# MarSaKi/VLN-BEVBert

Measured on AMD Instinct MI355X. Metric: pretrain_samples_per_sec, higher is better.
Workload: dtype bf16+fp32-residual

## Files before the change

### vln_bevbert_amd/csrc/attn_fwd2.hip

```cpp
#include "attn_mfma_common.h"

#define FWD2_THR 5.0f

typedef const __attribute__((address_space(4))) uint64_t* bb_cu64p;

__device__ __forceinline__ float drop_select(float p, uint64_t lane_mask) {
  return __builtin_amdgcn_inverse_ballot_w64(lane_mask) ? p : 0.f;
}
__device__ __forceinline__ float max3f(float a, float b, float c) { return fmaxf(fmaxf(a, b), c); }

#define F2_LD 72
#define F2_TILE (TK * F2_LD)
__device__ __forceinline__ int f2_off(int row, int chunk) { return row * F2_LD + (chunk << 3); }
__device__ __forceinline__ bf16x8 f2_frag_rows(const bf16_raw* tile, int t, int ks, int lane) {
  return as_bf16x8(*reinterpret_cast<const uint4*>(tile + f2_off(t * 16 + (lane & 15), ks * 4 + (lane >> 4))));
}
__device__ __forceinline__ bf16x8 f2_frag_tr(const bf16_raw* img, int row_lo, int row_hi, int col0, int lane) {
  const int i = lane & 15, col = col0 + 4 * (i & 3);
  const int rl = row_lo + (i >> 2), rh = row_hi + (i >> 2);
  const uint2 lo = lds_tr16(img + f2_off(rl, col >> 3) + (col & 7));
  const uint2 hi = lds_tr16(img + f2_off(rh, col >> 3) + (col & 7));
  return as_bf16x8(make_uint4(lo.x, lo.y, hi.x, hi.y));
}

template <int NW, bool DROP>
__global__ __launch_bounds__(64 * NW, 4) void attn_fwd2_kernel(AttnArgs a) {
  constexpr int QT = 2;
  constexpr int NT = 64 * NW;
  constexpr int CPT = (512 + NT - 1) / NT;
  __shared__ __attribute__((aligned(16))) bf16_raw s_k[2][F2_TILE];
  __shared__ __attribute__((aligned(16))) bf16_raw s_v[2][F2_TILE];
  __shared__ __attribute__((aligned(16))) float s_mask[2][TK];
  const int tid = threadIdx.x, lane = tid & 63, g = lane >> 4, c = lane & 15;
  const int w = __builtin_amdgcn_readfirstlane(tid >> 6);
  int blk, h, b;
  attn_decode_block(a, blk, h, b);
  const int qbase = blk * (16 * QT * NW) + w * (16 * QT);
  const bf16_raw* qp = (const bf16_raw*)a.q + (size_t)b * a.bsq + h * ATTN_D;
  const bf16_raw* kp = (const bf16_raw*)a.k + (size_t)b * a.bsk + h * ATTN_D;
  const bf16_raw* vp = (const bf16_raw*)a.v + (size_t)b * a.bsv + h * ATTN_D;
  const float sc2 = a.scale * LOG2E;
  const float inv_scale = 1.0f / a.scale;

  bf16x8 qf[QT][2];
  int qrow[QT];
#pragma unroll
  for (int qt = 0; qt < QT; ++qt) {
    qrow[qt] = qbase + qt * 16 + c;
    const int r = qrow[qt] < a.Lq ? qrow[qt] : a.Lq - 1;
#pragma unroll
    for (int ks = 0; ks < 2; ++ks) qf[qt][ks] = as_bf16x8(ld_frag_global(qp, a.ldq, r, ks * 32 + g * 8));
  }
  bb_cu64p wq[QT];
  if (DROP) {
#pragma unroll
    for (int qt = 0; qt < QT; ++qt) {
      int q16 = (qbase >> 4) + qt;
      q16 = q16 < a.nq16 ? q16 : a.nq16 - 1;
      wq[qt] = (bb_cu64p)(uintptr_t)(a.drop_bits + ((size_t)(b * a.nh + h) * a.nq16 + q16) * a.nk64 * 16);
    }
  }
  f32x4 oacc[QT][4];
  float m_run[QT], nm[QT], l_run[QT];
#pragma unroll
  for (int qt = 0; qt < QT; ++qt) {
    m_run[qt] = -INFINITY;
    nm[qt] = 0.f;
    l_run[qt] = 0.f;
#pragma unroll
    for (int dt = 0; dt < 4; ++dt) oacc[qt][dt] = (f32x4){0.f, 0.f, 0.f, 0.f};
  }

  auto mask_of = [&](int kv0) -> float {
    const int key = kv0 + tid;
    if (tid >= TK || key >= a.Lk) return -INFINITY;
    return a.key_mask ? a.key_mask[(size_t)b * a.Lk + key] * inv_scale : 0.f;
  };
  uint4 kreg[CPT], vreg[CPT];
  float mreg;
  auto stage_load = [&](int kv0) {
#pragma unroll
    for (int i = 0; i < CPT; ++i) {
      const int ch = tid + i * NT, row = ch >> 3, d0 = (ch & 7) * 8;
      kreg[i] = vreg[i] = make_uint4(0, 0, 0, 0);
      if (ch < 512 && kv0 + row < a.Lk) {
        kreg[i] = ld_frag_global(kp, a.ldk, kv0 + row, d0);
        vreg[i] = ld_frag_global(vp, a.ldv, kv0 + row, d0);
      }
    }
    mreg = mask_of(kv0);
  };
  auto stage_store = [&](int buf) {
#pragma unroll
    for (int i = 0; i < CPT; ++i) {
      const int ch = tid + i * NT, row = ch >> 3, d0 = (ch & 7) * 8;
      if (ch < 512) {
        *reinterpret_cast<uint4*>(s_k[buf] + f2_off(row, ch & 7)) = kreg[i];
        *reinterpret_cast<uint4*>(s_v[buf] + f2_off(row, ch & 7)) = vreg[i];
      }
    }
    if (tid < TK) s_mask[buf][tid] = mreg;
  };
  stage_load(0);
  stage_store(0);
  if (TK < a.Lk) stage_load(TK);
  __syncthreads();

  uint64_t kw[8];
#pragma unroll
  for (int i = 0; i < 8; ++i) kw[i] = DROP ? wq[0][i] : 0;
  for (int kv0 = 0, cur = 0; kv0 < a.Lk; kv0 += TK, cur ^= 1) {
    const bf16_raw* ck = s_k[cur];
    const bf16_raw* cv = s_v[cur];
    const float* cmask = s_mask[cur];
#pragma unroll
    for (int hh = 0; hh < 2; ++hh) {
      f32x4 sacc[QT][2];
#pragma unroll
      for (int tt = 0; tt < 2; ++tt) {
        const int t = 2 * hh + tt;
        const float4 mk = *reinterpret_cast<const float4*>(&cmask[t * 16 + g * 4]);
#pragma unroll
        for (int qt = 0; qt < QT; ++qt) sacc[qt][tt] = (f32x4){mk.x, mk.y, mk.z, mk.w};
#pragma unroll
        for (int ks = 0; ks < 2; ++ks) {
          const bf16x8 kf = f2_frag_rows(ck, t, ks, lane);
#pragma unroll
          for (int qt = 0; qt < QT; ++qt) sacc[qt][tt] = mfma16(kf, qf[qt][ks], sacc[qt][tt]);
        }
      }
      if (hh == 0 && kv0 + TK < a.Lk) {
        stage_store(cur ^ 1);
        if (kv0 + 2 * TK < a.Lk) stage_load(kv0 + 2 * TK);
      }
      float lm[QT];
      bool grow = false;
#pragma unroll
      for (int qt = 0; qt < QT; ++qt) {
        const f32x4 s0 = sacc[qt][0], s1 = sacc[qt][1];
        lm[qt] = max3f(max3f(s0[0], s0[1], s0[2]), max3f(s0[3], s1[0], s1[1]), fmaxf(s1[2], s1[3])) * sc2;
        grow |= lm[qt] > m_run[qt] + FWD2_THR;
      }
      if (__any(grow)) {
#pragma unroll
        for (int qt = 0; qt < QT; ++qt) {
          const float m_new = fmaxf(m_run[qt], quad_max(lm[qt]));
          const float nm_new = (m_new == -INFINITY) ? 0.f : -m_new;
          const float alpha = fast_exp2(m_run[qt] + nm_new);
          m_run[qt] = m_new;
          nm[qt] = nm_new;
          l_run[qt] *= alpha;
#pragma unroll
          for (int dt = 0; dt < 4; ++dt) oacc[qt][dt] *= alpha;
        }
      }
      bf16x8 pb[QT];
#pragma unroll
      for (int qt = 0; qt < QT; ++qt) {
        uint64_t kwn[8];
        if (DROP) {
          const int kvn = (qt + 1 < QT || hh == 0) ? kv0 : (kv0 + TK < a.Lk ? kv0 + TK : kv0);
          const int hn = qt + 1 < QT ? hh : hh ^ 1, qn = qt + 1 < QT ? qt + 1 : 0;
#pragma unroll
          for (int i = 0; i < 8; ++i) kwn[i] = wq[qn][(kvn >> 6) * 16 + hn * 8 + i];
          __builtin_amdgcn_sched_barrier(0);
        }
        float psum = 0.f;
#pragma unroll
        for (int tt = 0; tt < 2; ++tt)
#pragma unroll
          for (int r = 0; r < 4; ++r) {
            float p = fast_exp2(fmaf(sacc[qt][tt][r], sc2, nm[qt]));
            psum += p;
            if (DROP) p = drop_select(p, kw[tt * 4 + r]);
            sacc[qt][tt][r] = p;
          }
        l_run[qt] += psum;
        pb[qt] = pack_pair(sacc[qt][0], sacc[qt][1]);
        if (DROP) {
#pragma unroll
          for (int i = 0; i < 8; ++i) kw[i] = kwn[i];
        }
      }
#pragma unroll
      for (int dt = 0; dt < 4; ++dt) {
        const bf16x8 vf = f2_frag_tr(cv, 32 * hh + 4 * g, 32 * hh + 16 + 4 * g, dt * 16, lane);
#pragma unroll
        for (int qt = 0; qt < QT; ++qt) oacc[qt][dt] = mfma16(vf, pb[qt], oacc[qt][dt]);
      }

    }
    __syncthreads();
  }

  const float ks = DROP ? a.keep_scale : 1.0f;
#pragma unroll
  for (int qt = 0; qt < QT; ++qt) {
    const float l = quad_sum(l_run[qt]);
    const float inv = ks / l;
    if (qrow[qt] < a.Lq) {
      bf16_raw* op = (bf16_raw*)a.o + (size_t)b * a.bso + (size_t)qrow[qt] * a.ldo + h * ATTN_D;
#pragma unroll
      for (int dt = 0; dt < 4; ++dt)
        st4<bf16_raw>(op + dt * 16 + g * 4, make_float4(oacc[qt][dt][0] * inv, oacc[qt][dt][1] * inv,
                                                         oacc[qt][dt][2] * inv, oacc[qt][dt][3] * inv));
      if (a.lse && g == 0) a.lse[((size_t)b * a.nh + h) * a.Lq + qrow[qt]] = (log2f(l) - nm[qt]) * LN2;
    }
  }
}

template <int NW, bool DROP, int ABL = 0>
__global__ __launch_bounds__(64 * NW, 4) void attn_fwd3_kernel(AttnArgs a) {
  constexpr int QT = 2;
  constexpr int NT = 64 * NW;
  constexpr int CPT = (512 + NT - 1) / NT;
  __shared__ __attribute__((aligned(16))) bf16_raw s_k[2][F2_TILE];
  __shared__ __attribute__((aligned(16))) bf16_raw s_v[2][F2_TILE];
  __shared__ __attribute__((aligned(16))) float s_mask[2][TK];
  const int tid = threadIdx.x, lane = tid & 63, g = lane >> 4, c = lane & 15;
  const int w = __builtin_amdgcn_readfirstlane(tid >> 6);
  int blk, h, b;
  attn_decode_block(a, blk, h, b);
  const int qbase = blk * (16 * QT * NW) + w * (16 * QT);
  const bf16_raw* qp = (const bf16_raw*)a.q + (size_t)b * a.bsq + h * ATTN_D;
  const bf16_raw* kp = (const bf16_raw*)a.k + (size_t)b * a.bsk + h * ATTN_D;
  const bf16_raw* vp = (const bf16_raw*)a.v + (size_t)b * a.bsv + h * ATTN_D;
  const float sc2 = a.scale * LOG2E;
  const float inv_scale = 1.0f / a.scale;

  bf16x8 qf[QT][2];
  int qrow[QT];
#pragma unroll
  for (int qt = 0; qt < QT; ++qt) {
    qrow[qt] = qbase + qt * 16 + c;
    const int r = qrow[qt] < a.Lq ? qrow[qt] : a.Lq - 1;
#pragma unroll
    for (int ks = 0; ks < 2; ++ks) qf[qt][ks] = as_bf16x8(ld_frag_global(qp, a.ldq, r, ks * 32 + g * 8));
  }
  bb_cu64p wq[QT];
  if (DROP) {
#pragma unroll
    for (int qt = 0; qt < QT; ++qt) {
      int q16 = (qbase >> 4) + qt;
      q16 = q16 < a.nq16 ? q16 : a.nq16 - 1;
      wq[qt] = (bb_cu64p)(uintptr_t)(a.drop_bits + ((size_t)(b * a.nh + h) * a.nq16 + q16) * a.nk64 * 16);
    }
  }
  f32x4 oacc[QT][4];
  float m_run[QT], nm[QT], l_run[QT];
#pragma unroll
  for (int qt = 0; qt < QT; ++qt) {
    m_run[qt] = -INFINITY;
    nm[qt] = 0.f;
    l_run[qt] = 0.f;
#pragma unroll
    for (int dt = 0; dt < 4; ++dt) oacc[qt][dt] = (f32x4){0.f, 0.f, 0.f, 0.f};
  }

  auto mask_of = [&](int kv0) -> float {
    const int key = kv0 + tid;
    if (tid >= TK || key >= a.Lk) return -INFINITY;
    return a.key_mask ? a.key_mask[(size_t)b * a.Lk + key] * inv_scale : 0.f;
  };
  uint4 kreg[CPT], vreg[CPT];
  float mreg;
  auto stage_load = [&](int kv0) {
#pragma unroll
    for (int i = 0; i < CPT; ++i) {
      const int ch = tid + i * NT, row = ch >> 3, d0 = (ch & 7) * 8;
      kreg[i] = vreg[i] = make_uint4(0, 0, 0, 0);
      if (ch < 512 && kv0 + row < a.Lk) {
        kreg[i] = ld_frag_global(kp, a.ldk, kv0 + row, d0);
        vreg[i] = ld_frag_global(vp, a.ldv, kv0 + row, d0);
      }
    }
    mreg = mask_of(kv0);
  };
  auto stage_store = [&](int buf) {
#pragma unroll
    for (int i = 0; i < CPT; ++i) {
      const int ch = tid + i * NT, row = ch >> 3, d0 = (ch & 7) * 8;
      if (ch < 512) {
        *reinterpret_cast<uint4*>(s_k[buf] + f2_off(row, ch & 7)) = kreg[i];
        *reinterpret_cast<uint4*>(s_v[buf] + f2_off(row, ch & 7)) = vreg[i];
      }
    }
    if (tid < TK) s_mask[buf][tid] = mreg;
  };
  stage_load(0);
  stage_store(0);
  if (TK < a.Lk) stage_load(TK);
  __syncthreads();

  uint64_t kw[QT][16];
#pragma unroll
  for (int qt = 0; qt < QT; ++qt)
#pragma unroll
    for (int i = 0; i < 16; ++i) kw[qt][i] = DROP ? wq[qt][i] : 0;
  const int Lk_run = (ABL & 64) ? (a.Lk < TK ? a.Lk : TK) : a.Lk;
  for (int kv0 = 0, cur = 0; kv0 < Lk_run; kv0 += TK, cur ^= 1) {
    const bf16_raw* ck = s_k[cur];
    const bf16_raw* cv = s_v[cur];
    const float* cmask = s_mask[cur];
#pragma unroll
    for (int hh = 0; hh < 2; ++hh) {
      f32x4 sacc[QT][2];
#pragma unroll
      for (int tt = 0; tt < 2; ++tt) {
        const int t = 2 * hh + tt;
        const float4 mk = *reinterpret_cast<const float4*>(&cmask[t * 16 + g * 4]);
#pragma unroll
        for (int qt = 0; qt < QT; ++qt) sacc[qt][tt] = (f32x4){mk.x, mk.y, mk.z, mk.w};
#pragma unroll
        for (int ks = 0; ks < 2; ++ks) {
          const bf16x8 kf = f2_frag_rows(ck, t, ks, lane);
#pragma unroll
          for (int qt = 0; qt < QT; ++qt) if (!(ABL & 4)) sacc[qt][tt] = mfma16(kf, qf[qt][ks], sacc[qt][tt]);
        }
      }
      if (hh == 0 && kv0 + TK < a.Lk && !((ABL & 8) && kv0 > 0)) {
        stage_store(cur ^ 1);
        if (kv0 + 2 * TK < a.Lk) stage_load(kv0 + 2 * TK);
      }
#pragma unroll
      for (int qt = 0; qt < QT; ++qt)
#pragma unroll
        for (int tt = 0; tt < 2; ++tt)
#pragma unroll
          for (int r = 0; r < 4; ++r) sacc[qt][tt][r] = fmaf(sacc[qt][tt][r], sc2, nm[qt]);
      float lm[QT];
      bool grow = false;
#pragma unroll
      for (int qt = 0; qt < QT; ++qt) {
        const f32x4 s0 = sacc[qt][0], s1 = sacc[qt][1];
        lm[qt] = max3f(max3f(s0[0], s0[1], s0[2]), max3f(s0[3], s1[0], s1[1]), fmaxf(s1[2], s1[3]));
        grow |= (lm[qt] > FWD2_THR) | ((m_run[qt] == -INFINITY) & (lm[qt] > -INFINITY));
      }
      if ((ABL & 16) ? (kv0 == 0 && hh == 0) : __any(grow)) {
#pragma unroll
        for (int qt = 0; qt < QT; ++qt) {
          const float m_new = fmaxf(m_run[qt], quad_max(lm[qt]) - nm[qt]);
          const float nm_new = (m_new == -INFINITY) ? 0.f : -m_new;
          const float alpha = fast_exp2(m_run[qt] + nm_new);
          const float shift = nm_new - nm[qt];
          m_run[qt] = m_new;
          nm[qt] = nm_new;
          l_run[qt] *= alpha;
#pragma unroll
          for (int dt = 0; dt < 4; ++dt) oacc[qt][dt] *= alpha;
#pragma unroll
          for (int tt = 0; tt < 2; ++tt)
#pragma unroll
            for (int r = 0; r < 4; ++r) sacc[qt][tt][r] += shift;
        }
      }
      bf16x8 pb[QT];
#pragma unroll
      for (int qt = 0; qt < QT; ++qt) {
        float psum = 0.f;
#pragma unroll
        for (int tt = 0; tt < 2; ++tt)
#pragma unroll
          for (int r = 0; r < 4; ++r) {
            float p = (ABL & 1) ? sacc[qt][tt][r] : fast_exp2(sacc[qt][tt][r]);
            psum += p;
            if (DROP && !(ABL & 1)) {
              p = drop_select(p, kw[qt][(2 * hh + tt) * 4 + r]);
              asm("" : "+v"(p));
            }
            sacc[qt][tt][r] = p;
          }
        l_run[qt] += psum;
        pb[qt] = pack_pair(sacc[qt][0], sacc[qt][1]);
      }
#pragma unroll
      for (int dt = 0; dt < 4; ++dt) {
        const bf16x8 vf = f2_frag_tr(cv, 32 * hh + 4 * g, 32 * hh + 16 + 4 * g, dt * 16, lane);
#pragma unroll
        for (int qt = 0; qt < QT; ++qt) if (!(ABL & 2)) oacc[qt][dt] = mfma16(vf, pb[qt], oacc[qt][dt]);
      }

    }
    __builtin_amdgcn_sched_barrier(0);
    if (DROP) {
      const int kvn = kv0 + TK < a.Lk ? kv0 + TK : kv0;
      bb_cu64p w0 = wq[0] + (kvn >> 6) * 16, w1 = wq[1] + (kvn >> 6) * 16;
      asm volatile("s_waitcnt lgkmcnt(0)" : "+s"(w0), "+s"(w1) : : "memory");
#pragma unroll
      for (int i = 0; i < 16; ++i) { kw[0][i] = w0[i]; kw[1][i] = w1[i]; }
    } else {
      asm volatile("s_waitcnt lgkmcnt(0)" : : : "memory");
    }
    __builtin_amdgcn_s_barrier();
    asm volatile("" : : : "memory");
  }

  const float ks = DROP ? a.keep_scale : 1.0f;
#pragma unroll
  for (int qt = 0; qt < QT; ++qt) {
    const float l = quad_sum(l_run[qt]);
    const float inv = ks / l;
    if (qrow[qt] < a.Lq) {
      bf16_raw* op = (bf16_raw*)a.o + (size_t)b * a.bso + (size_t)qrow[qt] * a.ldo + h * ATTN_D;
#pragma unroll
      for (int dt = 0; dt < 4; ++dt)
        st4<bf16_raw>(op + dt * 16 + g * 4, make_float4(oacc[qt][dt][0] * inv, oacc[qt][dt][1] * inv,
                                                         oacc[qt][dt][2] * inv, oacc[qt][dt][3] * inv));
      if (a.lse && g == 0) a.lse[((size_t)b * a.nh + h) * a.Lq + qrow[qt]] = (log2f(l) - nm[qt]) * LN2;
    }
  }
}

template <int LANE0> __device__ __forceinline__ void put_words4(uint32_t& lo, uint32_t& hi, uint64_t m0, uint64_t m1,
                                                              uint64_t m2, uint64_t m3) {
  asm volatile("s_nop 3\n\t"
               "v_writelane_b32 %0, %2, %10\n\tv_writelane_b32 %1, %3, %10\n\t"
               "v_writelane_b32 %0, %4, %11\n\tv_writelane_b32 %1, %5, %11\n\t"
               "v_writelane_b32 %0, %6, %12\n\tv_writelane_b32 %1, %7, %12\n\t"
               "v_writelane_b32 %0, %8, %13\n\tv_writelane_b32 %1, %9, %13"
               : "+v"(lo), "+v"(hi)
               : "s"((uint32_t)m0), "s"((uint32_t)(m0 >> 32)), "s"((uint32_t)m1), "s"((uint32_t)(m1 >> 32)),
                 "s"((uint32_t)m2), "s"((uint32_t)(m2 >> 32)), "s"((uint32_t)m3), "s"((uint32_t)(m3 >> 32)),
                 "n"(LANE0), "n"(LANE0 + 1), "n"(LANE0 + 2), "n"(LANE0 + 3));
}

template <bool WITH_B>
__global__ __launch_bounds__(256) void attn_drop_bits_kernel(AttnArgs a, uint64_t* bits_f, uint64_t* bits_b, uint32_t* bits_l) {
  constexpr int NQT = WITH_B ? 4 : 1;
  const int lane = threadIdx.x & 63, g = lane >> 4, c = lane & 15;
  const int wave = blockIdx.x * 4 + (threadIdx.x >> 6), nwaves = gridDim.x * 4;
  const uint32_t key = bb_salted(a.drop_key, a.salt);
  const uint32_t thr_hi = a.drop_thr << 16;
  const int nqg = a.nq16 / NQT, per_bh = nqg * a.nk64, total = a.B * a.nh * per_bh;
  for (int gtask = wave; gtask < total; gtask += nwaves) {
    const int bh = gtask / per_bh, rem = gtask - bh * per_bh, qg = rem / a.nk64, k64 = rem - qg * a.nk64;
    uint32_t wl0 = 0, wl1 = 0;
#pragma unroll 1
   for (int qt = 0; qt < NQT; ++qt) {
    const int q16 = qg * NQT + qt;
    const int task = (bh * a.nq16 + q16) * a.nk64 + k64;
    const int q = q16 * 16 + c;
    const uint32_t rbase = (uint32_t)(((uint32_t)bh * a.Lq + (q < a.Lq ? q : a.Lq - 1)) * (uint32_t)a.Lk2);
    uint32_t mine = 0;
    uint32_t flo = 0, fhi = 0;
#pragma unroll
    for (int t = 0; t < 4; ++t) {
      const uint32_t pr = (rbase + (uint32_t)(k64 * 64 + t * 16 + g * 4)) >> 1;
      const uint32_t b0 = bb_pair_bits(key, pr), b1 = bb_pair_bits(key, pr + 1);
      const bool k0 = (b0 << 16) >= thr_hi, k1 = b0 >= thr_hi, k2 = (b1 << 16) >= thr_hi, k3 = b1 >= thr_hi;
      const uint64_t m0 = __ballot(k0), m1 = __ballot(k1), m2 = __ballot(k2), m3 = __ballot(k3);
      if (t == 0) put_words4<0>(flo, fhi, m0, m1, m2, m3);
      if (t == 1) put_words4<4>(flo, fhi, m0, m1, m2, m3);
      if (t == 2) put_words4<8>(flo, fhi, m0, m1, m2, m3);
      if (t == 3) put_words4<12>(flo, fhi, m0, m1, m2, m3);
      if (WITH_B) {
        const uint32_t nib = (k0 ? 1u : 0u) | (k1 ? 2u : 0u) | (k2 ? 4u : 0u) | (k3 ? 8u : 0u);
        mine |= nib << (4 * t);
      }
    }
    if (lane < 16) bits_f[(size_t)task * 16 + lane] = ((uint64_t)fhi << 32) | flo;
    if (WITH_B) {
      uint32_t blo = 0, bhi = 0;
      uint32_t got[4];
#pragma unroll
      for (int rp = 0; rp < 4; ++rp)
        got[rp] = (uint32_t)__builtin_amdgcn_ds_bpermute(((c >> 2) * 16 + 4 * g + rp) << 2, (int)mine) >> (c & 3);
#define BB_B_WORDS(T) put_words4<4 * T>(blo, bhi, __ballot((got[0] >> (4 * T)) & 1u), __ballot((got[1] >> (4 * T)) & 1u), \
                                        __ballot((got[2] >> (4 * T)) & 1u), __ballot((got[3] >> (4 * T)) & 1u));
      BB_B_WORDS(0) BB_B_WORDS(1) BB_B_WORDS(2) BB_B_WORDS(3)
#undef BB_B_WORDS
      if (lane < 16) {
        const int t = lane >> 2, rp = lane & 3;
        const size_t wi = ((((size_t)bh * (a.nq16 >> 1) + (q16 >> 1)) * a.nk64 + k64) * 2 + (q16 & 1)) * 16 + t * 4 + rp;
        bits_b[wi] = ((uint64_t)bhi << 32) | blo;
      }
      uint32_t ev = mine & 0x5555u, od = (mine >> 1) & 0x5555u;
      ev = (ev | (ev >> 1)) & 0x3333u; od = (od | (od >> 1)) & 0x3333u;
      ev = (ev | (ev >> 2)) & 0x0f0fu; od = (od | (od >> 2)) & 0x0f0fu;
      ev = (ev | (ev >> 4)) & 0x00ffu; od = (od | (od >> 4)) & 0x00ffu;
      wl0 |= ((ev & 15u) | ((od & 15u) << 16)) << (4 * qt);
      wl1 |= ((ev >> 4) | ((od >> 4) << 16)) << (4 * qt);
    }
   }
    if (WITH_B) {
      uint32_t* dst = bits_l + (((size_t)bh * nqg + qg) * a.nk64 + k64) * 128 + lane;
      dst[0] = wl0;
      dst[64] = wl1;
    }
  }
}

int attn_drop_bits(const AttnArgs& a, uint64_t* bits_f, uint64_t* bits_b, uint32_t* bits_l, hipStream_t st) {
  const bool with_b = bits_b != nullptr && bits_l != nullptr && a.bias == nullptr && a.Lk > 256 && a.Lk <= 448;
  const int total = a.B * a.nh * (with_b ? a.nq16 / 4 : a.nq16) * a.nk64;
  int nb = (total + 3) / 4;
  if (nb > 8192) nb = 8192;
  if (with_b) hipLaunchKernelGGL(attn_drop_bits_kernel<true>, dim3(nb), dim3(256), 0, st, a, bits_f, bits_b, bits_l);
  else hipLaunchKernelGGL(attn_drop_bits_kernel<false>, dim3(nb), dim3(256), 0, st, a, bits_f, bits_b, bits_l);
  BB_CHECK_LAUNCH("attn_drop_bits");
  return BB_OK;
}

template <int NW>
static int launch_fwd2(const AttnArgs& a_in, hipStream_t st) {
  AttnArgs a = a_in;
  a.nblk = (a.Lq + 32 * NW - 1) / (32 * NW);
  const dim3 grid((unsigned)a.nblk * a.nh * a.B);
  static const int var = [] { const char* v = getenv("BEVBERT_FWD_VAR"); return v ? atoi(v) : 1; }();
  if (var == 0) {
    if (a.drop_p > 0.f) hipLaunchKernelGGL((attn_fwd2_kernel<NW, true>), grid, dim3(64 * NW), 0, st, a);
    else hipLaunchKernelGGL((attn_fwd2_kernel<NW, false>), grid, dim3(64 * NW), 0, st, a);
  } else {
    static const int abl = [] { const char* v = getenv("BEVBERT_FWD_ABL"); return v ? atoi(v) : 0; }();
    if (abl && a.drop_p > 0.f && NW == 4) {
      switch (abl) {
        case 1: hipLaunchKernelGGL((attn_fwd3_kernel<4, true, 1>), grid, dim3(256), 0, st, a); return BB_OK;
        case 2: hipLaunchKernelGGL((attn_fwd3_kernel<4, true, 2>), grid, dim3(256), 0, st, a); return BB_OK;
        case 4: hipLaunchKernelGGL((attn_fwd3_kernel<4, true, 4>), grid, dim3(256), 0, st, a); return BB_OK;
        case 6: hipLaunchKernelGGL((attn_fwd3_kernel<4, true, 6>), grid, dim3(256), 0, st, a); return BB_OK;
        case 7: hipLaunchKernelGGL((attn_fwd3_kernel<4, true, 7>), grid, dim3(256), 0, st, a); return BB_OK;
        case 8: hipLaunchKernelGGL((attn_fwd3_kernel<4, true, 8>), grid, dim3(256), 0, st, a); return BB_OK;
        case 16: hipLaunchKernelGGL((attn_fwd3_kernel<4, true, 16>), grid, dim3(256), 0, st, a); return BB_OK;
        case 17: hipLaunchKernelGGL((attn_fwd3_kernel<4, true, 17>), grid, dim3(256), 0, st, a); return BB_OK;
        case 31: hipLaunchKernelGGL((attn_fwd3_kernel<4, true, 31>), grid, dim3(256), 0, st, a); return BB_OK;
        case 64: hipLaunchKernelGGL((attn_fwd3_kernel<4, true, 64>), grid, dim3(256), 0, st, a); return BB_OK;
        case 95: hipLaunchKernelGGL((attn_fwd3_kernel<4, true, 95>), grid, dim3(256), 0, st, a); return BB_OK;
        default: break;
      }
    }
    if (a.drop_p > 0.f) hipLaunchKernelGGL((attn_fwd3_kernel<NW, true>), grid, dim3(64 * NW), 0, st, a);
    else hipLaunchKernelGGL((attn_fwd3_kernel<NW, false>), grid, dim3(64 * NW), 0, st, a);
  }
  BB_CHECK_LAUNCH("attn_fwd(mfma, gen 2)");
  return BB_OK;
}

bool attn_fwd2_supported(const AttnArgs& a) { return a.bias == nullptr && (a.drop_p <= 0.f || a.drop_bits != nullptr); }

int attn_fwd2(const AttnArgs& a, hipStream_t st) {
  BB_REQUIRE(attn_mfma_operands_aligned(a, false), "attention (MFMA path): " ATTN_MFMA_ALIGN_MSG);
  static const int force = [] { const char* v = getenv("BEVBERT_FWD2_NW"); return v ? atoi(v) : 0; }();
  if (force == 7) return launch_fwd2<7>(a, st);
  if (force == 8) return launch_fwd2<8>(a, st);
  return launch_fwd2<4>(a, st);
}
```

### vln_bevbert_amd/csrc/splat.hip

```cpp
#include "common.h"

#define MAX_CELLS 1024
#define MAX_POINTS 24576

struct LiftArgs {
  const float* depths;
  const float* T_c2w;
  const float* T_w2c;
  const float* S_w2c;
  const float* pix;
  const float* points;
  const uint8_t* pmask;
  int V, hw;
  float depth_scale;
  int P, dim;
  float res, half, y_clip;
  int* cell;
  int* order;
  int* cell_start;
};

__device__ __forceinline__ int cell_of(float ex, float ey, float ez, bool dropped, int dim, float res, float half,
                                       float y_clip) {
  const float fx = rintf(__fadd_rn(__fdiv_rn(ex, res), half));
  const float fz = rintf(__fadd_rn(__fdiv_rn(ez, res), half));
  const float fd = (float)dim;
  const bool outside = (fx >= fd) | (fz >= fd) | (fx < 0.f) | (fz < 0.f);
  if (dropped | outside | (ey > y_clip)) return -1;
  return dim * (int)fz + (int)fx;
}

#define LIFT_WAVES 16
#define LIFT_THREADS (LIFT_WAVES * 64)
template <int MODE>
__global__ __launch_bounds__(LIFT_THREADS) void bev_bin_sort_kernel(LiftArgs a) {
  __shared__ short s_cell[MAX_POINTS];
  __shared__ int s_cnt[MAX_CELLS + 1];
  const int b = blockIdx.x, tid = threadIdx.x;
  const int K = a.dim * a.dim;
  for (int c = tid; c <= K; c += LIFT_THREADS) s_cnt[c] = 0;
  __syncthreads();

  for (int p = tid; p < a.P; p += LIFT_THREADS) {
    int cid;
    if (MODE == 0) {
      const int hw2 = a.hw * a.hw;
      const int v = p / hw2, r = (p - v * hw2) / a.hw, u = p % a.hw;
      const float z = __fmul_rn(a.depths[(size_t)b * a.P + p], a.depth_scale);
      const float x = __fmul_rn(z, a.pix[u]);
      const float y = __fmul_rn(z, a.pix[r]);
      const float* T = a.T_c2w + ((size_t)b * a.V + v) * 16;
      float w[3];
#pragma unroll
      for (int i = 0; i < 3; ++i)
        w[i] = __fadd_rn(__fadd_rn(__fadd_rn(__fmul_rn(T[i * 4 + 0], x), __fmul_rn(T[i * 4 + 1], y)),
                                   __fmul_rn(T[i * 4 + 2], z)),
                         T[i * 4 + 3]);
      const float* S = a.S_w2c + (size_t)b * 3;
      const float p0 = __fsub_rn(w[0], S[0]), p1 = __fsub_rn(w[1], S[1]), p2 = __fsub_rn(w[2], S[2]);
      const float* R = a.T_w2c + (size_t)b * 16;
      float e[3];
#pragma unroll
      for (int i = 0; i < 3; ++i)
        e[i] = __fadd_rn(__fadd_rn(__fadd_rn(__fmul_rn(R[i * 4 + 0], p0), __fmul_rn(R[i * 4 + 1], p1)),
                                   __fmul_rn(R[i * 4 + 2], p2)),
                         R[i * 4 + 3]);
      cid = cell_of(e[0], e[1], e[2], z == 0.f, a.dim, a.res, a.half, a.y_clip);
    } else {
      const float* q = a.points + ((size_t)b * a.P + p) * 3;
      cid = cell_of(q[0], q[1], q[2], a.pmask[(size_t)b * a.P + p] != 0, a.dim, a.res, a.half, a.y_clip);
    }
    s_cell[p] = (short)cid;
    a.cell[(size_t)b * a.P + p] = cid;
    if (cid >= 0) atomicAdd(&s_cnt[cid], 1);
  }
  __syncthreads();

  if (tid < 64) {
    const int per = (K + 63) / 64;
    const int c0 = tid * per;
    int sum = 0;
    for (int i = 0; i < per; ++i)
      if (c0 + i < K) sum += s_cnt[c0 + i];
    int incl = sum;
#pragma unroll
    for (int o = 1; o < 64; o <<= 1) {
      int t = __shfl_up(incl, o, 64);
      if (tid >= o) incl += t;
    }
    int run = incl - sum;
    for (int i = 0; i < per; ++i)
      if (c0 + i < K) {
        const int n = s_cnt[c0 + i];
        s_cnt[c0 + i] = run;
        run += n;
      }
    if (tid == 63) s_cnt[K] = incl;
  }
  __syncthreads();
  for (int c = tid; c <= K; c += LIFT_THREADS) a.cell_start[(size_t)b * (K + 1) + c] = s_cnt[c];

  __shared__ int s_wbase[LIFT_WAVES][MAX_CELLS + 1];
  const int lane = tid & 63, wv = tid >> 6;
  for (int c = tid; c < LIFT_WAVES * (MAX_CELLS + 1); c += LIFT_THREADS) (&s_wbase[0][0])[c] = 0;
  __syncthreads();
  const int per_wave = ((a.P + LIFT_THREADS - 1) / LIFT_THREADS) * 64;
  const int pw0 = wv * per_wave;
  for (int p = pw0 + lane; p < pw0 + per_wave && p < a.P; p += 64) {
    const int cid = s_cell[p];
    if (cid >= 0) atomicAdd(&s_wbase[wv][cid], 1);
  }
  __syncthreads();
  for (int c = tid; c < K; c += LIFT_THREADS) {
    int base = s_cnt[c];
#pragma unroll
    for (int w = 0; w < LIFT_WAVES; ++w) {
      const int n = s_wbase[w][c];
      s_wbase[w][c] = base;
      base += n;
    }
  }
  __syncthreads();
  int* dst = a.order + (size_t)b * a.P;
  const unsigned long long lt = lane == 0 ? 0ull : (~0ull >> (64 - lane));
  for (int p0 = pw0; p0 < pw0 + per_wave && p0 < a.P; p0 += 64) {
    const int p = p0 + lane;
    const int cid = p < a.P ? (int)s_cell[p] : -1;
    unsigned long long todo = __ballot(cid >= 0);
    while (todo) {
      const int leader = __builtin_ctzll(todo);
      const int c0 = __shfl(cid, leader, 64);
      const unsigned long long same = __ballot(cid == c0);
      const int base = s_wbase[wv][c0];
      if (cid == c0) dst[base + __builtin_popcountll(same & lt)] = p;
      if (lane == leader) s_wbase[wv][c0] = base + __builtin_popcountll(same);
      todo &= ~same;
    }
  }
}

template <typename TI, typename TO>
__global__ __launch_bounds__(256) void bev_splat_mean_kernel(const TI* __restrict__ feat, const int* __restrict__ order,
                                                             const int* __restrict__ cell_start, TO* __restrict__ out,
                                                             int P, int K, int C,
                                                             const uint8_t* __restrict__ sem_ids,
                                                             const double* __restrict__ sem_dense,
                                                             int S, uint8_t* __restrict__ out_sem,
                                                             uint8_t* __restrict__ out_sem_mask,
                                                             const int* __restrict__ sample_rows,
                                                             int R) {
  const int cellg = blockIdx.x;
  const int b = cellg / K, cell = cellg - b * K;
  const int P0 = P / R;
  const int* rows = sample_rows != nullptr ? sample_rows + (size_t)b * R : nullptr;
  auto src_point = [&](int p) -> size_t {
    if (rows == nullptr) return (size_t)b * P + p;
    if (R == 1) return (size_t)rows[0] * P0 + p;
    const int r = p / P0;
    return (size_t)rows[r] * P0 + (p - r * P0);
  };
  const int s0 = cell_start[(size_t)b * (K + 1) + cell];
  const int n = cell_start[(size_t)b * (K + 1) + cell + 1] - s0;
  const int* ord = order + (size_t)b * P + s0;
  const float inv_denominator = (float)(n > 1 ? n : 1);

  for (int c4 = threadIdx.x; c4 * 4 < C; c4 += blockDim.x) {
    float4 acc = make_float4(0.f, 0.f, 0.f, 0.f);
    int i = 0;
    for (; i + 4 <= n; i += 4) {
      const int p0 = ord[i], p1 = ord[i + 1], p2 = ord[i + 2], p3 = ord[i + 3];
      const float4 v0 = ld4<TI>(feat + src_point(p0) * C + c4 * 4);
      const float4 v1 = ld4<TI>(feat + src_point(p1) * C + c4 * 4);
      const float4 v2 = ld4<TI>(feat + src_point(p2) * C + c4 * 4);
      const float4 v3 = ld4<TI>(feat + src_point(p3) * C + c4 * 4);
      acc.x = __fadd_rn(__fadd_rn(__fadd_rn(__fadd_rn(acc.x, v0.x), v1.x), v2.x), v3.x);
      acc.y = __fadd_rn(__fadd_rn(__fadd_rn(__fadd_rn(acc.y, v0.y), v1.y), v2.y), v3.y);
      acc.z = __fadd_rn(__fadd_rn(__fadd_rn(__fadd_rn(acc.z, v0.z), v1.z), v2.z), v3.z);
      acc.w = __fadd_rn(__fadd_rn(__fadd_rn(__fadd_rn(acc.w, v0.w), v1.w), v2.w), v3.w);
    }
    for (; i < n; ++i) {
      const float4 v = ld4<TI>(feat + src_point(ord[i]) * C + c4 * 4);
      acc.x = __fadd_rn(acc.x, v.x); acc.y = __fadd_rn(acc.y, v.y);
      acc.z = __fadd_rn(acc.z, v.z); acc.w = __fadd_rn(acc.w, v.w);
    }
    acc.x = __fdiv_rn(acc.x, inv_denominator); acc.y = __fdiv_rn(acc.y, inv_denominator);
    acc.z = __fdiv_rn(acc.z, inv_denominator); acc.w = __fdiv_rn(acc.w, inv_denominator);
    st4<TO>(out + (size_t)cellg * C + c4 * 4, acc);
  }

  if (out_sem != nullptr) {
    int any = 0;
    for (int c = threadIdx.x; c < S; c += blockDim.x) {
      uint8_t flag = 0;
      if (sem_ids != nullptr) {
        for (int i = 0; i < n; ++i) flag |= (uint8_t)(sem_ids[src_point(ord[i])] == (uint8_t)c);
      } else {
        const double* sb = sem_dense + (size_t)b * P * S;
        double acc = 0.0;
        for (int i = 0; i < n; ++i) acc += sb[(size_t)ord[i] * S + c];
        flag = (uint8_t)(acc / (double)(n > 1 ? n : 1) > 0.0);
      }
      out_sem[(size_t)cellg * S + c] = flag;
      any |= flag;
    }
    any = __syncthreads_or(any);
    if (threadIdx.x == 0) out_sem_mask[cellg] = (uint8_t)(any != 0);
  }
}

BEVBERT_API int bevbert_bev_lift_bin(const float* depths, const float* T_c2w, const float* T_w2c, const float* S_w2c,
                                     const float* pix_scale, int B, int V, int hw, float depth_scale, int dim,
                                     float res, float y_clip, int* cell, int* order, int* cell_start,
                                     hipStream_t stream) {
  const int P = V * hw * hw;
  BB_REQUIRE(B > 0 && P > 0 && P <= MAX_POINTS, "bev_lift_bin: P=%d out of range (max %d)", P, MAX_POINTS);
  BB_REQUIRE(dim > 0 && dim * dim <= MAX_CELLS, "bev_lift_bin: dim=%d too large", dim);
  LiftArgs a;
  memset(&a, 0, sizeof(a));
  a.depths = depths; a.T_c2w = T_c2w; a.T_w2c = T_w2c; a.S_w2c = S_w2c; a.pix = pix_scale;
  a.V = V; a.hw = hw; a.depth_scale = depth_scale; a.P = P; a.dim = dim; a.res = res;
  a.half = (float)(dim - 1) / 2.0f; a.y_clip = y_clip;
  a.cell = cell; a.order = order; a.cell_start = cell_start;
  hipLaunchKernelGGL(bev_bin_sort_kernel<0>, dim3(B), dim3(LIFT_THREADS), 0, stream, a);
  BB_CHECK_LAUNCH("bev_lift_bin");
  return BB_OK;
}

BEVBERT_API int bevbert_bev_bin_points(const float* points, const uint8_t* drop_mask, int B, int P, int dim, float res,
                                       float y_clip, int* cell, int* order, int* cell_start, hipStream_t stream) {
  BB_REQUIRE(B > 0 && P > 0 && P <= MAX_POINTS, "bev_bin_points: P=%d out of range (max %d)", P, MAX_POINTS);
  BB_REQUIRE(dim > 0 && dim * dim <= MAX_CELLS, "bev_bin_points: dim=%d too large", dim);
  LiftArgs a;
  memset(&a, 0, sizeof(a));
  a.points = points; a.pmask = drop_mask; a.P = P; a.dim = dim; a.res = res;
  a.half = (float)(dim - 1) / 2.0f; a.y_clip = y_clip;
  a.cell = cell; a.order = order; a.cell_start = cell_start;
  hipLaunchKernelGGL(bev_bin_sort_kernel<1>, dim3(B), dim3(LIFT_THREADS), 0, stream, a);
  BB_CHECK_LAUNCH("bev_bin_points");
  return BB_OK;
}

template <typename TI, typename TO>
static int launch_splat(const void* feat, const int* order, const int* cell_start, void* out, int B, int P, int K,
                        int C, const uint8_t* sem_ids, const double* sem_dense, int S, uint8_t* out_sem,
                        uint8_t* out_sem_mask, const int* sample_rows, int R, hipStream_t stream) {
  const int threads = (C / 4 >= 192) ? 192 : ((C / 4 + 63) / 64) * 64;
  hipLaunchKernelGGL((bev_splat_mean_kernel<TI, TO>), dim3(B * K), dim3(threads < 64 ? 64 : threads), 0, stream,
                     (const TI*)feat, order, cell_start, (TO*)out, P, K, C, sem_ids, sem_dense, S, out_sem,
                     out_sem_mask, sample_rows, R);
  BB_CHECK_LAUNCH("bev_splat_mean");
  return BB_OK;
}

BEVBERT_API int bevbert_bev_splat_mean(const void* feat, int feat_dtype, const int* order, const int* cell_start,
                                       void* out, int out_dtype, int B, int P, int K, int C, const uint8_t* sem_ids,
                                       const double* sem_dense, int S, uint8_t* out_sem, uint8_t* out_sem_mask,
                                       const int* sample_rows, int rows_per_sample, hipStream_t stream) {
  BB_REQUIRE(C % 4 == 0, "bev_splat_mean: C=%d must be a multiple of 4", C);
  const int R = rows_per_sample < 1 ? 1 : rows_per_sample;
  BB_REQUIRE(R == 1 || sample_rows != nullptr, "bev_splat_mean: rows_per_sample=%d needs sample_rows", R);
  BB_REQUIRE(P % R == 0, "bev_splat_mean: P=%d is not a multiple of rows_per_sample=%d", P, R);
  BB_REQUIRE(sample_rows == nullptr || sem_dense == nullptr,
             "bev_splat_mean: sample_rows indexes feat / sem_ids stores; dense semantics are per batch");
  BB_REQUIRE(out_sem == nullptr || (sem_ids != nullptr) != (sem_dense != nullptr),
             "bev_splat_mean: exactly one of sem_ids / sem_dense when semantics are requested");
#define GO(TI, TO) \
  return launch_splat<TI, TO>(feat, order, cell_start, out, B, P, K, C, sem_ids, sem_dense, S, out_sem, out_sem_mask, sample_rows, R, stream)
  if (feat_dtype == BB_F32 && out_dtype == BB_F32) GO(float, float);
  if (feat_dtype == BB_F32 && out_dtype == BB_BF16) GO(float, bf16_raw);
  if (feat_dtype == BB_BF16 && out_dtype == BB_F32) GO(bf16_raw, float);
  if (feat_dtype == BB_BF16 && out_dtype == BB_BF16) GO(bf16_raw, bf16_raw);
  if (feat_dtype == BB_F16 && out_dtype == BB_F32) GO(_Float16, float);
  if (feat_dtype == BB_F16 && out_dtype == BB_BF16) GO(_Float16, bf16_raw);
  if (feat_dtype == BB_F16 && out_dtype == BB_F16) GO(_Float16, _Float16);
#undef GO
  bb_set_error("bev_splat_mean: unsupported dtype pair (%d -> %d)", feat_dtype, out_dtype);
  return BB_EUNSUPPORTED;
}
```

Baseline: 3703.

## Parallelize BEV bin-sort across point chunks and streamline dropout-bit packing

The BEV bin-sort kernel now launches one block per (batch, point chunk) rather than one block per batch. Each block recomputes cell ids for all points to get global counts, then ranks its own points inside each wave by intersecting one ballot per cell-id bit, and scatters the order entries directly. This trades redundant per-block cell computation for much more parallelism than a single block per sample. Separately, the attention dropout-bit kernel's WITH_B path is restructured: transposed and lane-packed masks are built with carry-add lane-bit accumulation and bpermute plus bit-swizzles, replacing per-tile ballots and shift cascades.

Result: no change. 3694 (-0.3%).

```diff
diff --git a/vln_bevbert_amd/csrc/attn_fwd2.hip b/vln_bevbert_amd/csrc/attn_fwd2.hip
--- a/vln_bevbert_amd/csrc/attn_fwd2.hip
+++ b/vln_bevbert_amd/csrc/attn_fwd2.hip
@@ -424,6 +424,80 @@
                  "n"(LANE0), "n"(LANE0 + 1), "n"(LANE0 + 2), "n"(LANE0 + 3));
 }
 
+template <int LANE0> __device__ __forceinline__ void put_words4_lane_bits(uint32_t& lo, uint32_t& hi, uint32_t& ev, uint32_t& od,
+                                                                        uint64_t m0, uint64_t m1, uint64_t m2, uint64_t m3) {
+  asm volatile("s_nop 3\n\t"
+               "v_writelane_b32 %[lo], %[m0l], %[l0]\n\tv_writelane_b32 %[hi], %[m0h], %[l0]\n\t"
+               "v_writelane_b32 %[lo], %[m1l], %[l1]\n\tv_writelane_b32 %[hi], %[m1h], %[l1]\n\t"
+               "v_writelane_b32 %[lo], %[m2l], %[l2]\n\tv_writelane_b32 %[hi], %[m2h], %[l2]\n\t"
+               "v_writelane_b32 %[lo], %[m3l], %[l3]\n\tv_writelane_b32 %[hi], %[m3h], %[l3]\n\t"
+               "v_addc_co_u32_e64 %[od], vcc, %[od], %[od], %[m3]\n\t"
+               "v_addc_co_u32_e64 %[ev], vcc, %[ev], %[ev], %[m2]\n\t"
+               "v_addc_co_u32_e64 %[od], vcc, %[od], %[od], %[m1]\n\t"
+               "v_addc_co_u32_e64 %[ev], vcc, %[ev], %[ev], %[m0]"
+               : [lo] "+v"(lo), [hi] "+v"(hi), [ev] "+v"(ev), [od] "+v"(od)
+               : [m0l] "s"((uint32_t)m0), [m0h] "s"((uint32_t)(m0 >> 32)), [m1l] "s"((uint32_t)m1),
+                 [m1h] "s"((uint32_t)(m1 >> 32)), [m2l] "s"((uint32_t)m2), [m2h] "s"((uint32_t)(m2 >> 32)),
+                 [m3l] "s"((uint32_t)m3), [m3h] "s"((uint32_t)(m3 >> 32)), [m0] "s"(m0), [m1] "s"(m1), [m2] "s"(m2),
+                 [m3] "s"(m3), [l0] "n"(LANE0), [l1] "n"(LANE0 + 1), [l2] "n"(LANE0 + 2), [l3] "n"(LANE0 + 3)
+               : "vcc");
+}
+
+template <int QT, int T>
+__device__ __forceinline__ void drop_bits_step(uint32_t key, uint32_t thr_hi, uint32_t elem0, uint32_t& flo, uint32_t& fhi,
+                                               uint32_t& ev, uint32_t& od) {
+  const uint32_t pr = (elem0 + (uint32_t)(T * 16)) >> 1;
+  const uint32_t b0 = bb_pair_bits(key, pr), b1 = bb_pair_bits(key, pr + 1);
+  const bool k0 = (b0 << 16) >= thr_hi, k1 = b0 >= thr_hi, k2 = (b1 << 16) >= thr_hi, k3 = b1 >= thr_hi;
+  put_words4_lane_bits<16 * QT + 4 * T>(flo, fhi, ev, od, __ballot(k0), __ballot(k1), __ballot(k2), __ballot(k3));
+}
+
+template <int QT>
+__device__ __forceinline__ void drop_bits_tile(const AttnArgs& a, uint32_t key, uint32_t thr_hi, int bh, int q16, int k64,
+                                               int g, int c, uint32_t& flo, uint32_t& fhi, uint32_t (&acc)[2][2]) {
+  const int q = q16 * 16 + c;
+  const uint32_t rbase = (uint32_t)(((uint32_t)bh * a.Lq + (q < a.Lq ? q : a.Lq - 1)) * (uint32_t)a.Lk2);
+  const uint32_t elem0 = rbase + (uint32_t)(k64 * 64 + g * 4);
+  drop_bits_step<QT, 3>(key, thr_hi, elem0, flo, fhi, acc[1][0], acc[1][1]);
+  drop_bits_step<QT, 2>(key, thr_hi, elem0, flo, fhi, acc[1][0], acc[1][1]);
+  drop_bits_step<QT, 1>(key, thr_hi, elem0, flo, fhi, acc[0][0], acc[0][1]);
+  drop_bits_step<QT, 0>(key, thr_hi, elem0, flo, fhi, acc[0][0], acc[0][1]);
+}
+
+__device__ __forceinline__ void drop_bits_task_fbl(const AttnArgs& a, uint32_t key, uint32_t thr_hi, int bh, int qg, int k64,
+                                                   int lane, uint64_t* bits_f, uint64_t* bits_b, uint32_t* bits_l) {
+  const int g = lane >> 4, c = lane & 15;
+  uint32_t flo = 0, fhi = 0;
+  uint32_t acc[2][2] = {{0, 0}, {0, 0}};
+  drop_bits_tile<3>(a, key, thr_hi, bh, qg * 4 + 3, k64, g, c, flo, fhi, acc);
+  drop_bits_tile<2>(a, key, thr_hi, bh, qg * 4 + 2, k64, g, c, flo, fhi, acc);
+  drop_bits_tile<1>(a, key, thr_hi, bh, qg * 4 + 1, k64, g, c, flo, fhi, acc);
+  drop_bits_tile<0>(a, key, thr_hi, bh, qg * 4 + 0, k64, g, c, flo, fhi, acc);
+  const int q16 = qg * 4 + g, j = c;
+  const int task = (bh * a.nq16 + q16) * a.nk64 + k64;
+  bits_f[(size_t)task * 16 + j] = ((uint64_t)fhi << 32) | flo;
+
+  const int rp = lane & 3, quad = (lane & ~3) << 2;
+  uint32_t xlo = 0, xhi = 0;
+#pragma unroll
+  for (int i = 0; i < 4; ++i) {
+    const uint32_t slo = (uint32_t)__builtin_amdgcn_ds_bpermute(quad + 4 * i, (int)flo);
+    const uint32_t shi = (uint32_t)__builtin_amdgcn_ds_bpermute(quad + 4 * i, (int)fhi);
+    xlo |= ((slo >> rp) & 0x11111111u) << i;
+    xhi |= ((shi >> rp) & 0x11111111u) << i;
+  }
+  uint64_t x = ((uint64_t)xhi << 32) | xlo;
+  uint64_t sw = ((x >> 12) ^ x) & 0x0000F0F00000F0F0ull;
+  x ^= sw ^ (sw << 12);
+  sw = ((x >> 24) ^ x) & 0x00000000FF00FF00ull;
+  x ^= sw ^ (sw << 24);
+  const size_t wi = ((((size_t)bh * (a.nq16 >> 1) + (q16 >> 1)) * a.nk64 + k64) * 2 + (q16 & 1)) * 16 + j;
+  bits_b[wi] = x;
+  uint32_t* dst = bits_l + (((size_t)bh * (a.nq16 / 4) + qg) * a.nk64 + k64) * 128 + lane;
+  dst[0] = acc[0][0] | (acc[0][1] << 16);
+  dst[64] = acc[1][0] | (acc[1][1] << 16);
+}
+
 template <bool WITH_B>
 __global__ __launch_bounds__(256) void attn_drop_bits_kernel(AttnArgs a, uint64_t* bits_f, uint64_t* bits_b, uint32_t* bits_l) {
   constexpr int NQT = WITH_B ? 4 : 1;
@@ -434,14 +508,13 @@
   const int nqg = a.nq16 / NQT, per_bh = nqg * a.nk64, total = a.B * a.nh * per_bh;
   for (int gtask = wave; gtask < total; gtask += nwaves) {
     const int bh = gtask / per_bh, rem = gtask - bh * per_bh, qg = rem / a.nk64, k64 = rem - qg * a.nk64;
-    uint32_t wl0 = 0, wl1 = 0;
-#pragma unroll 1
-   for (int qt = 0; qt < NQT; ++qt) {
-    const int q16 = qg * NQT + qt;
-    const int task = (bh * a.nq16 + q16) * a.nk64 + k64;
-    const int q = q16 * 16 + c;
+    if (WITH_B) {
+      drop_bits_task_fbl(a, key, thr_hi, bh, qg, k64, lane, bits_f, bits_b, bits_l);
+      continue;
+    }
+    const int task = (bh * a.nq16 + qg) * a.nk64 + k64;
+    const int q = qg * 16 + c;
     const uint32_t rbase = (uint32_t)(((uint32_t)bh * a.Lq + (q < a.Lq ? q : a.Lq - 1)) * (uint32_t)a.Lk2);
-    uint32_t mine = 0;
     uint32_t flo = 0, fhi = 0;
 #pragma unroll
     for (int t = 0; t < 4; ++t) {
@@ -453,40 +526,8 @@
       if (t == 1) put_words4<4>(flo, fhi, m0, m1, m2, m3);
       if (t == 2) put_words4<8>(flo, fhi, m0, m1, m2, m3);
       if (t == 3) put_words4<12>(flo, fhi, m0, m1, m2, m3);
-      if (WITH_B) {
-        const uint32_t nib = (k0 ? 1u : 0u) | (k1 ? 2u : 0u) | (k2 ? 4u : 0u) | (k3 ? 8u : 0u);
-        mine |= nib << (4 * t);
-      }
     }
     if (lane < 16) bits_f[(size_t)task * 16 + lane] = ((uint64_t)fhi << 32) | flo;
-    if (WITH_B) {
-      uint32_t blo = 0, bhi = 0;
-      uint32_t got[4];
-#pragma unroll
-      for (int rp = 0; rp < 4; ++rp)
-        got[rp] = (uint32_t)__builtin_amdgcn_ds_bpermute(((c >> 2) * 16 + 4 * g + rp) << 2, (int)mine) >> (c & 3);
-#define BB_B_WORDS(T) put_words4<4 * T>(blo, bhi, __ballot((got[0] >> (4 * T)) & 1u), __ballot((got[1] >> (4 * T)) & 1u), \
-                                        __ballot((got[2] >> (4 * T)) & 1u), __ballot((got[3] >> (4 * T)) & 1u));
-      BB_B_WORDS(0) BB_B_WORDS(1) BB_B_WORDS(2) BB_B_WORDS(3)
-#undef BB_B_WORDS
-      if (lane < 16) {
-        const int t = lane >> 2, rp = lane & 3;
-        const size_t wi = ((((size_t)bh * (a.nq16 >> 1) + (q16 >> 1)) * a.nk64 + k64) * 2 + (q16 & 1)) * 16 + t * 4 + rp;
-        bits_b[wi] = ((uint64_t)bhi << 32) | blo;
-      }
-      uint32_t ev = mine & 0x5555u, od = (mine >> 1) & 0x5555u;
-      ev = (ev | (ev >> 1)) & 0x3333u; od = (od | (od >> 1)) & 0x3333u;
-      ev = (ev | (ev >> 2)) & 0x0f0fu; od = (od | (od >> 2)) & 0x0f0fu;
-      ev = (ev | (ev >> 4)) & 0x00ffu; od = (od | (od >> 4)) & 0x00ffu;
-      wl0 |= ((ev & 15u) | ((od & 15u) << 16)) << (4 * qt);
-      wl1 |= ((ev >> 4) | ((od >> 4) << 16)) << (4 * qt);
-    }
-   }
-    if (WITH_B) {
-      uint32_t* dst = bits_l + (((size_t)bh * nqg + qg) * a.nk64 + k64) * 128 + lane;
-      dst[0] = wl0;
-      dst[64] = wl1;
-    }
   }
 }
 
diff --git a/vln_bevbert_amd/csrc/splat.hip b/vln_bevbert_amd/csrc/splat.hip
--- a/vln_bevbert_amd/csrc/splat.hip
+++ b/vln_bevbert_amd/csrc/splat.hip
@@ -30,113 +30,138 @@
   return dim * (int)fz + (int)fx;
 }
 
+struct LiftIn { float x, y, z; bool dropped; };
+
+template <int MODE>
+__device__ __forceinline__ LiftIn lift_load(const LiftArgs& a, int b, int p) {
+  LiftIn in = {0.f, 0.f, 0.f, true};
+  if (p >= a.P) return in;
+  if (MODE == 0) {
+    in.z = a.depths[(size_t)b * a.P + p];
+  } else {
+    const float* q = a.points + ((size_t)b * a.P + p) * 3;
+    in.x = q[0]; in.y = q[1]; in.z = q[2];
+    in.dropped = a.pmask[(size_t)b * a.P + p] != 0;
+  }
+  return in;
+}
+
+template <int MODE>
+__device__ __forceinline__ int lift_cell(const LiftArgs& a, int b, int p, const LiftIn& in) {
+  if (MODE == 0) {
+    const int hw2 = a.hw * a.hw;
+    const int v = p / hw2, r = (p - v * hw2) / a.hw, u = p % a.hw;
+    const float z = __fmul_rn(in.z, a.depth_scale);
+    const float x = __fmul_rn(z, a.pix[u]);
+    const float y = __fmul_rn(z, a.pix[r]);
+    const float* T = a.T_c2w + ((size_t)b * a.V + v) * 16;
+    float w[3];
+#pragma unroll
+    for (int i = 0; i < 3; ++i)
+      w[i] = __fadd_rn(__fadd_rn(__fadd_rn(__fmul_rn(T[i * 4 + 0], x), __fmul_rn(T[i * 4 + 1], y)),
+                                 __fmul_rn(T[i * 4 + 2], z)),
+                       T[i * 4 + 3]);
+    const float* S = a.S_w2c + (size_t)b * 3;
+    const float p0 = __fsub_rn(w[0], S[0]), p1 = __fsub_rn(w[1], S[1]), p2 = __fsub_rn(w[2], S[2]);
+    const float* R = a.T_w2c + (size_t)b * 16;
+    float e[3];
+#pragma unroll
+    for (int i = 0; i < 3; ++i)
+      e[i] = __fadd_rn(__fadd_rn(__fadd_rn(__fmul_rn(R[i * 4 + 0], p0), __fmul_rn(R[i * 4 + 1], p1)),
+                                 __fmul_rn(R[i * 4 + 2], p2)),
+                       R[i * 4 + 3]);
+    return cell_of(e[0], e[1], e[2], z == 0.f, a.dim, a.res, a.half, a.y_clip);
+  }
+  return cell_of(in.x, in.y, in.z, in.dropped, a.dim, a.res, a.half, a.y_clip);
+}
+
 #define LIFT_WAVES 16
 #define LIFT_THREADS (LIFT_WAVES * 64)
+#define LIFT_CHUNK LIFT_THREADS
+#define LIFT_CELL_BITS 10
 template <int MODE>
 __global__ __launch_bounds__(LIFT_THREADS) void bev_bin_sort_kernel(LiftArgs a) {
-  __shared__ short s_cell[MAX_POINTS];
-  __shared__ int s_cnt[MAX_CELLS + 1];
-  const int b = blockIdx.x, tid = threadIdx.x;
+  static_assert(MAX_CELLS == (1 << LIFT_CELL_BITS), "one ballot per bit of the cell id");
+  __shared__ int s_before[MAX_CELLS];
+  __shared__ int s_rest[MAX_CELLS + 1];
+  __shared__ unsigned short s_wave[LIFT_WAVES][MAX_CELLS];
+  const int b = blockIdx.x, chunk = blockIdx.y, tid = threadIdx.x;
+  const int lane = tid & 63, wv = tid >> 6;
   const int K = a.dim * a.dim;
-  for (int c = tid; c <= K; c += LIFT_THREADS) s_cnt[c] = 0;
+  const int chunk_p0 = chunk * LIFT_CHUNK, p_own = chunk_p0 + tid;
+  for (int c = tid; c < K; c += LIFT_THREADS) {
+    s_before[c] = 0;
+    s_rest[c] = 0;
+#pragma unroll
+    for (int w = 0; w < LIFT_WAVES; ++w) s_wave[w][c] = 0;
+  }
   __syncthreads();
 
-  for (int p = tid; p < a.P; p += LIFT_THREADS) {
-    int cid;
-    if (MODE == 0) {
-      const int hw2 = a.hw * a.hw;
-      const int v = p / hw2, r = (p - v * hw2) / a.hw, u = p % a.hw;
-      const float z = __fmul_rn(a.depths[(size_t)b * a.P + p], a.depth_scale);
-      const float x = __fmul_rn(z, a.pix[u]);
-      const float y = __fmul_rn(z, a.pix[r]);
-      const float* T = a.T_c2w + ((size_t)b * a.V + v) * 16;
-      float w[3];
-#pragma unroll
-      for (int i = 0; i < 3; ++i)
-        w[i] = __fadd_rn(__fadd_rn(__fadd_rn(__fmul_rn(T[i * 4 + 0], x), __fmul_rn(T[i * 4 + 1], y)),
-                                   __fmul_rn(T[i * 4 + 2], z)),
-                         T[i * 4 + 3]);
-      const float* S = a.S_w2c + (size_t)b * 3;
-      const float p0 = __fsub_rn(w[0], S[0]), p1 = __fsub_rn(w[1], S[1]), p2 = __fsub_rn(w[2], S[2]);
-      const float* R = a.T_w2c + (size_t)b * 16;
-      float e[3];
-#pragma unroll
-      for (int i = 0; i < 3; ++i)
-        e[i] = __fadd_rn(__fadd_rn(__fadd_rn(__fmul_rn(R[i * 4 + 0], p0), __fmul_rn(R[i * 4 + 1], p1)),
-                                   __fmul_rn(R[i * 4 + 2], p2)),
-                         R[i * 4 + 3]);
-      cid = cell_of(e[0], e[1], e[2], z == 0.f, a.dim, a.res, a.half, a.y_clip);
-    } else {
-      const float* q = a.points + ((size_t)b * a.P + p) * 3;
-      cid = cell_of(q[0], q[1], q[2], a.pmask[(size_t)b * a.P + p] != 0, a.dim, a.res, a.half, a.y_clip);
-    }
-    s_cell[p] = (short)cid;
-    a.cell[(size_t)b * a.P + p] = cid;
-    if (cid >= 0) atomicAdd(&s_cnt[cid], 1);
-  }
+  int mine = -1;
+  for (int pb = tid; pb < a.P; pb += 4 * LIFT_THREADS) {
+    LiftIn in[4];
+#pragma unroll
+    for (int j = 0; j < 4; ++j) in[j] = lift_load<MODE>(a, b, pb + j * LIFT_THREADS);
+#pragma unroll
+    for (int j = 0; j < 4; ++j) {
+      const int p = pb + j * LIFT_THREADS;
+      if (p < a.P) {
+        const int cid = lift_cell<MODE>(a, b, p, in[j]);
+        if (p == p_own) {
+          mine = cid;
+          a.cell[(size_t)b * a.P + p] = cid;
+        }
+        if (cid >= 0) atomicAdd(p < chunk_p0 ? &s_before[cid] : &s_rest[cid], 1);
+      }
+    }
+  }
+
+  unsigned long long same = __ballot(mine >= 0);
+#pragma unroll
+  for (int bit = 0; bit < LIFT_CELL_BITS; ++bit) {
+    const bool set = (mine >> bit) & 1;
+    const unsigned long long m = __ballot(set);
+    same &= set ? m : ~m;
+  }
+  const unsigned long long lt = lane == 0 ? 0ull : (~0ull >> (64 - lane));
+  const int rank = __builtin_popcountll(same & lt);
+  if (mine >= 0 && rank == 0) s_wave[wv][mine] = (unsigned short)__builtin_popcountll(same);
   __syncthreads();
 
-  if (tid < 64) {
+  for (int c = tid; c < K; c += LIFT_THREADS) {
+    int run = 0;
+#pragma unroll
+    for (int w = 0; w < LIFT_WAVES; ++w) {
+      const int n = s_wave[w][c];
+      s_wave[w][c] = (unsigned short)run;
+      run += n;
+    }
+  }
+  if (wv == LIFT_WAVES - 1) {
     const int per = (K + 63) / 64;
-    const int c0 = tid * per;
+    const int c0 = lane * per;
     int sum = 0;
     for (int i = 0; i < per; ++i)
-      if (c0 + i < K) sum += s_cnt[c0 + i];
+      if (c0 + i < K) sum += s_before[c0 + i] + s_rest[c0 + i];
     int incl = sum;
 #pragma unroll
     for (int o = 1; o < 64; o <<= 1) {
       int t = __shfl_up(incl, o, 64);
-      if (tid >= o) incl += t;
+      if (lane >= o) incl += t;
     }
     int run = incl - sum;
     for (int i = 0; i < per; ++i)
       if (c0 + i < K) {
-        const int n = s_cnt[c0 + i];
-        s_cnt[c0 + i] = run;
+        const int n = s_before[c0 + i] + s_rest[c0 + i];
+        s_rest[c0 + i] = run;
         run += n;
       }
-    if (tid == 63) s_cnt[K] = incl;
+    if (lane == 63) s_rest[K] = incl;
   }
   __syncthreads();
-  for (int c = tid; c <= K; c += LIFT_THREADS) a.cell_start[(size_t)b * (K + 1) + c] = s_cnt[c];
-
-  __shared__ int s_wbase[LIFT_WAVES][MAX_CELLS + 1];
-  const int lane = tid & 63, wv = tid >> 6;
-  for (int c = tid; c < LIFT_WAVES * (MAX_CELLS + 1); c += LIFT_THREADS) (&s_wbase[0][0])[c] = 0;
-  __syncthreads();
-  const int per_wave = ((a.P + LIFT_THREADS - 1) / LIFT_THREADS) * 64;
-  const int pw0 = wv * per_wave;
-  for (int p = pw0 + lane; p < pw0 + per_wave && p < a.P; p += 64) {
-    const int cid = s_cell[p];
-    if (cid >= 0) atomicAdd(&s_wbase[wv][cid], 1);
-  }
-  __syncthreads();
-  for (int c = tid; c < K; c += LIFT_THREADS) {
-    int base = s_cnt[c];
-#pragma unroll
-    for (int w = 0; w < LIFT_WAVES; ++w) {
-      const int n = s_wbase[w][c];
-      s_wbase[w][c] = base;
-      base += n;
-    }
-  }
-  __syncthreads();
-  int* dst = a.order + (size_t)b * a.P;
-  const unsigned long long lt = lane == 0 ? 0ull : (~0ull >> (64 - lane));
-  for (int p0 = pw0; p0 < pw0 + per_wave && p0 < a.P; p0 += 64) {
-    const int p = p0 + lane;
-    const int cid = p < a.P ? (int)s_cell[p] : -1;
-    unsigned long long todo = __ballot(cid >= 0);
-    while (todo) {
-      const int leader = __builtin_ctzll(todo);
-      const int c0 = __shfl(cid, leader, 64);
-      const unsigned long long same = __ballot(cid == c0);
-      const int base = s_wbase[wv][c0];
-      if (cid == c0) dst[base + __builtin_popcountll(same & lt)] = p;
-      if (lane == leader) s_wbase[wv][c0] = base + __builtin_popcountll(same);
-      todo &= ~same;
-    }
-  }
+  if (chunk == 0)
+    for (int c = tid; c <= K; c += LIFT_THREADS) a.cell_start[(size_t)b * (K + 1) + c] = s_rest[c];
+  if (mine >= 0) a.order[(size_t)b * a.P + s_rest[mine] + s_before[mine] + s_wave[wv][mine] + rank] = p_own;
 }
 
 template <typename TI, typename TO>
@@ -221,7 +246,7 @@
   a.V = V; a.hw = hw; a.depth_scale = depth_scale; a.P = P; a.dim = dim; a.res = res;
   a.half = (float)(dim - 1) / 2.0f; a.y_clip = y_clip;
   a.cell = cell; a.order = order; a.cell_start = cell_start;
-  hipLaunchKernelGGL(bev_bin_sort_kernel<0>, dim3(B), dim3(LIFT_THREADS), 0, stream, a);
+  hipLaunchKernelGGL(bev_bin_sort_kernel<0>, dim3(B, (P + LIFT_CHUNK - 1) / LIFT_CHUNK), dim3(LIFT_THREADS), 0, stream, a);
   BB_CHECK_LAUNCH("bev_lift_bin");
   return BB_OK;
 }
@@ -235,7 +260,7 @@
   a.points = points; a.pmask = drop_mask; a.P = P; a.dim = dim; a.res = res;
   a.half = (float)(dim - 1) / 2.0f; a.y_clip = y_clip;
   a.cell = cell; a.order = order; a.cell_start = cell_start;
-  hipLaunchKernelGGL(bev_bin_sort_kernel<1>, dim3(B), dim3(LIFT_THREADS), 0, stream, a);
+  hipLaunchKernelGGL(bev_bin_sort_kernel<1>, dim3(B, (P + LIFT_CHUNK - 1) / LIFT_CHUNK), dim3(LIFT_THREADS), 0, stream, a);
   BB_CHECK_LAUNCH("bev_bin_points");
   return BB_OK;
 }
```
